# frodik13/gstreamer-vit-tracker

Measured on NVIDIA B200. Metric: 1080p tracked frames/s, higher is better.
Workload: dtype bf16x3 (split bf16 operands, fp32 accumulate)

## Files before the change

gstreamer_vit_tracker_b200/csrc/attention_tc.cu:

```cuda
#include "tc_common.cuh"
#include "vt_internal.h"

namespace vt {

using namespace tc;

constexpr int kDh = 64;
constexpr int kQTile = 128;
constexpr int kKeyChunk = 64;
constexpr int kNChunks = kNTok / kKeyChunk;
constexpr int kQBytes = kQTile * kDh * 2;
constexpr int kKBytes = kNTok * kDh * 2;
constexpr int kVBytes = kDh * kNTok * 2;
constexpr int kPBytes = kQTile * kKeyChunk * 2;
constexpr uint32_t kTmemCols = 512;
constexpr uint32_t kColO = 320;
constexpr uint32_t kColA = 128;
constexpr int kSoftmaxWarps = 16, kSoftmaxThreads = kSoftmaxWarps * 32;
constexpr int kAttThreads = kSoftmaxThreads + 32;
constexpr int kColGroups = kSoftmaxThreads / kQTile;
constexpr int kKeysPerThread = kKeyChunk / kColGroups;

template <int NSPLIT>
struct AttSmem {
    static constexpr int kParts = NSPLIT == 3 ? 2 : 1;
    static constexpr int kQK = kParts * (kQBytes + kKBytes);
    static constexpr int kP = kParts * kPBytes;
    static constexpr int kRegion1 = kQK > kP ? kQK : kP;
    static constexpr int kV = kParts * kVBytes;
    static constexpr int kW2 = kParts * kAttChainW * 128;
    static constexpr int kTotal = kRegion1 + kV + kW2 + 1024;
};

__device__ __forceinline__ void softmax_bar_sync() { asm volatile("bar.sync 1, %0;" ::"n"(kSoftmaxThreads) : "memory"); }

template <int NSPLIT>
__global__ void __launch_bounds__(kAttThreads, 1)
attention_tc_kernel(const __grid_constant__ TcAttentionPlan mp, __nv_bfloat16* __restrict__ out_hi, __nv_bfloat16* __restrict__ out_lo, int D,
                    int heads, int* err, unsigned long long* trace, int dup) {
    const CUtensorMap &mQhi = mp.mQhi, &mQlo = mp.mQlo, &mKhi = mp.mKhi, &mKlo = mp.mKlo, &mVhi = mp.mVhi, &mVlo = mp.mVlo;
    extern __shared__ uint8_t smem_raw[];
    __shared__ __align__(8) uint64_t bar_qk, bar_k1, bar_v, bar_s, p_full[kNChunks], bar_o, bar_w2, bar_a2, bar_o2;
    __shared__ uint32_t tmem_base_s;
    __shared__ float red[kColGroups][kQTile];
    __shared__ unsigned long long* trace_slot;
    using SM = AttSmem<NSPLIT>;
    constexpr int P = SM::kParts;
    uint8_t* smem = reinterpret_cast<uint8_t*>((reinterpret_cast<uintptr_t>(smem_raw) + 1023) & ~uintptr_t(1023));
    uint8_t* sQ = smem;
    uint8_t* sK = smem + P * kQBytes;
    uint8_t* sV = smem + SM::kRegion1;
    uint8_t* sW2 = sV + SM::kV;

    const int tid = threadIdx.x, warp = tid >> 5, lane = tid & 31;
    const bool ctrl = warp == kSoftmaxWarps;
    const int row = (warp & 3) * 32 + lane;
    const int g = (warp >> 2) & 3;
    constexpr int kQTiles = (kNTok + kQTile - 1) / kQTile;
    const int replica = blockIdx.x / kQTiles;
    const bool st_hi = !dup || replica == 0, st_lo = P == 2 && (!dup || replica == 1);
    const bool chain = mp.chain != 0;
    const int q0 = (blockIdx.x % kQTiles) * kQTile, h = blockIdx.y, b = blockIdx.z;
    const int bh = b * heads + h;
    const bool q_ok = q0 + row < kNTok;
    bool ok = true;
    TraceRec tr;
    tr.begin(&trace_slot, trace, 10);

    if (tid == 0) {
        mbar_init(&bar_qk, 1), mbar_init(&bar_k1, 1), mbar_init(&bar_v, 1), mbar_init(&bar_s, 1), mbar_init(&bar_o, 1);
        mbar_init(&bar_w2, 1), mbar_init(&bar_a2, kSoftmaxWarps), mbar_init(&bar_o2, 1);
        for (int c = 0; c < kNChunks; ++c) mbar_init(&p_full[c], kSoftmaxWarps);
        fence_barrier_init();
    }
    if (ctrl) {
        if (elect_one_sync()) {
            tma_prefetch_desc(&mQhi), tma_prefetch_desc(&mKhi), tma_prefetch_desc(&mVhi);
            if (P == 2) tma_prefetch_desc(&mQlo), tma_prefetch_desc(&mKlo), tma_prefetch_desc(&mVlo);
        }
        tmem_alloc(&tmem_base_s, kTmemCols);
        tmem_relinquish();
    }
    tcgen05_fence_before();
    __syncthreads();
    if (chain && ctrl && elect_one_sync()) {
// ... 8 lines not shown
    pdl_wait();
    if (tid == 0) tr.mark(2);
    pdl_launch_dependents();

    if (ctrl) {
        if (elect_one_sync()) {
            constexpr int kHalfK = kNTok / 2, kHalfKBytes = kHalfK * kDh * 2;
            mbar_arrive_expect_tx(&bar_qk, P * (kQBytes + kHalfKBytes));
            tma_load_3d(sQ, &mQhi, &bar_qk, 0, q0, bh);
            tma_load_3d(sK, &mKhi, &bar_qk, 0, 0, bh);
            if (P == 2) tma_load_3d(sQ + kQBytes, &mQlo, &bar_qk, 0, q0, bh), tma_load_3d(sK + kKBytes, &mKlo, &bar_qk, 0, 0, bh);
            mbar_arrive_expect_tx(&bar_k1, P * kHalfKBytes);
            tma_load_3d(sK + kHalfKBytes, &mKhi, &bar_k1, 0, kHalfK, bh);
            if (P == 2) tma_load_3d(sK + kKBytes + kHalfKBytes, &mKlo, &bar_k1, 0, kHalfK, bh);
            mbar_arrive_expect_tx(&bar_v, P * kVBytes);
            for (int c = 0; c < kNChunks; ++c) {
                tma_load_3d(sV + c * (P * kDh * 128), &mVhi, &bar_v, c * kKeyChunk, 0, bh);
                if (P == 2) tma_load_3d(sV + c * (P * kDh * 128) + kDh * 128, &mVlo, &bar_v, c * kKeyChunk, 0, bh);
            }
            ok &= mbar_wait(&bar_qk, 0);
            tcgen05_fence_after();
            const uint64_t dQ = umma_desc_sw128(smem_u32(sQ)), dK = umma_desc_sw128(smem_u32(sK));
            constexpr int kHalf = kNTok / 2;
            constexpr uint32_t idescS = umma_idesc_h<NSPLIT == 2>(kQTile, kHalf);
            constexpr uint64_t kLoQ = kQBytes >> 4, kLoK = kKBytes >> 4, kK2 = (kHalf * 128) >> 4;
#pragma unroll
            for (int half = 0; half < 2; ++half) {
                if (half) {
                    ok &= mbar_wait(&bar_k1, 0);
                    tcgen05_fence_after();
                }
#pragma unroll
                for (int k = 0; k < kDh / 16; ++k) {
                    const uint64_t qh = dQ + 2 * k, kh = dK + 2 * k + half * kK2;
                    umma_bf16(tmem + half * kHalf, qh, kh, idescS, k != 0);
                    if (NSPLIT == 3) {
                        umma_bf16(tmem + half * kHalf, qh, kh + kLoK, idescS, 1);
                        umma_bf16(tmem + half * kHalf, qh + kLoQ, kh, idescS, 1);
                    }
                }
            }
            umma_commit(&bar_s);
            const uint64_t dV = umma_desc_sw128(smem_u32(sV));
            constexpr uint32_t idesc = umma_idesc_h<NSPLIT == 2>(kQTile, kDh), idesc2n = umma_idesc_h<NSPLIT == 2>(kQTile, 2 * kDh);
            constexpr uint64_t kBlkV = (uint64_t)(P * kDh * 128) >> 4;
            ok &= mbar_wait(&bar_v, 0);
            for (int c = 0; c < kNChunks; ++c) {
                ok &= mbar_wait(&p_full[c], 0);
                tcgen05_fence_after();
#pragma unroll
                for (int k = 0; k < kKeyChunk / 16; ++k) {
                    const uint32_t ph = tmem + c * kKeyChunk + k * kKeysPerThread;
                    const uint64_t vh = dV + c * kBlkV + 2 * k;
                    if (NSPLIT == 3) {
                        umma_bf16_ta(tmem + kColO, ph, vh, idesc2n, (c | k) != 0);
                        umma_bf16_ta(tmem + kColO, ph + 8, vh, idesc, 1);
                    } else {
                        umma_bf16_ta(tmem + kColO, ph, vh, idesc, (c | k) != 0);
                    }
                }
            }
            umma_commit(&bar_o);
            if (chain) {
                ok &= mbar_wait(&bar_w2, 0);
                ok &= mbar_wait(&bar_a2, 0);
                tcgen05_fence_after();
                const uint64_t dW = umma_desc_sw128(smem_u32(sW2));
                constexpr uint32_t idescW = umma_idesc_h<NSPLIT == 2>(kQTile, kAttChainW), idescW2 = umma_idesc_h<NSPLIT == 2>(kQTile, 2 * kAttChainW);
#pragma unroll
                for (int k = 0; k < kDh / 16; ++k) {
                    const uint32_t ah = tmem + kColA + k * 16;
                    if (NSPLIT == 3) {
                        umma_bf16_ta(tmem, ah, dW + 2 * k, idescW2, k != 0);
                        umma_bf16_ta(tmem, ah + 8, dW + 2 * k, idescW, 1);
                    } else {
                        umma_bf16_ta(tmem, ah, dW + 2 * k, idescW, k != 0);
                    }
                }
                umma_commit(&bar_o2);
            }
        }
        __syncwarp();
    } else {
        ok &= mbar_wait(&bar_s, 0);
        tcgen05_fence_after();
        if (tid == 0) tr.mark(4);
        const uint32_t lane_addr = tmem + ((uint32_t)((warp & 3) * 32) << 16);
        const float k2 = 1.4426950408889634f / sqrtf((float)kDh);
        float mx = -INFINITY;
        const uint32_t col0 = lane_addr + g * kKeysPerThread;
        uint32_t r[2][16];
        if (q_ok) {
            tmem_ld_32x16_issue(col0, r[0]);
#pragma unroll
            for (int c = 0; c < kNChunks; ++c) {
                tmem_ld_wait(r[c & 1]);
                if (c + 1 < kNChunks) tmem_ld_32x16_issue(col0 + (c + 1) * kKeyChunk, r[(c + 1) & 1]);
#pragma unroll
                for (int j = 0; j < 16; ++j) mx = fmaxf(mx, __uint_as_float(r[c & 1][j]));
            }
            tmem_ld_32x16_issue(col0, r[0]);
        }
        red[g][row] = mx;
        softmax_bar_sync();
        mx = fmaxf(fmaxf(red[0][row], red[1][row]), fmaxf(red[2][row], red[3][row]));
        if (tid == 0) tr.mark(5);
        const float mk = mx * k2;
        float sum = 0.f;
#pragma unroll
        for (int c = 0; c < kNChunks; ++c) {
            uint32_t hi[8], lo[8];
            if (q_ok) {
                tmem_ld_wait(r[c & 1]);
                if (c + 1 < kNChunks) tmem_ld_32x16_issue(col0 + (c + 1) * kKeyChunk, r[(c + 1) & 1]);
#pragma unroll
                for (int j = 0; j < 16; j += 2) {
                    const float e0 = ex2_approx(fmaf(__uint_as_float(r[c & 1][j]), k2, -mk));
                    const float e1 = ex2_approx(fmaf(__uint_as_float(r[c & 1][j + 1]), k2, -mk));
                    sum += e0;
                    sum += e1;
                    split2_h<NSPLIT == 2>(e0, e1, hi[j >> 1], lo[j >> 1]);
                }
            }
            if (q_ok) {
                tmem_st_32x8(col0 + c * kKeyChunk, hi);
                if (P == 2) tmem_st_32x8(col0 + c * kKeyChunk + 8, lo);
                tmem_st_wait();
            }
            tcgen05_fence_before();
            __syncwarp();
            if (lane == 0) mbar_arrive(&p_full[c]);
            if (tid == 0 && c == 0) tr.mark(6);
        }
        if (tid == 0) tr.mark(7);
        red[g][row] = sum;
        softmax_bar_sync();
        sum = (red[0][row] + red[1][row]) + (red[2][row] + red[3][row]);

        ok &= mbar_wait(&bar_o, 0);
        tcgen05_fence_after();
        {
            const float inv = q_ok ? 1.f / sum : 0.f;
            float v[16];
            tmem_ld_32x16(lane_addr + kColO + g * 16, v);
            if (NSPLIT == 3) {
                float hl[16];
                tmem_ld_32x16(lane_addr + kColO + kDh + g * 16, hl);
#pragma unroll
                for (int j = 0; j < 16; ++j) v[j] += hl[j];
            }
            uint32_t hi[8], lo[8];
#pragma unroll
            for (int j = 0; j < 16; j += 2) split2_h<NSPLIT == 2>(v[j] * inv, v[j + 1] * inv, hi[j >> 1], lo[j >> 1]);
            if (chain) {
                tmem_st_32x8(lane_addr + kColA + g * 16, hi);
                if (P == 2) tmem_st_32x8(lane_addr + kColA + g * 16 + 8, lo);
                tmem_st_wait();
            } else {
#pragma unroll
                for (int j = 0; j < 2; ++j) {
                    const int off = row * 128 + (((2 * g + j) ^ (row & 7)) << 4);
                    *reinterpret_cast<uint4*>(smem + off) = make_uint4(hi[4 * j], hi[4 * j + 1], hi[4 * j + 2], hi[4 * j + 3]);
                    if (P == 2) *reinterpret_cast<uint4*>(smem + kPBytes + off) = make_uint4(lo[4 * j], lo[4 * j + 1], lo[4 * j + 2], lo[4 * j + 3]);
                }
            }
        }
        if (chain) {
            tcgen05_fence_before();
            __syncwarp();
            if (lane == 0) mbar_arrive(&bar_a2);
            ok &= mbar_wait(&bar_o2, 0);
            tcgen05_fence_after();
            constexpr int CW = kAttChainW / kColGroups;
            float v[CW];
            tmem_ld_cols(lane_addr + g * CW, v);
            if (NSPLIT == 3) {
                float hl[CW];
                tmem_ld_cols(lane_addr + kAttChainW + g * CW, hl);
#pragma unroll
                for (int j = 0; j < CW; ++j) v[j] += hl[j];
            }
            uint8_t* prow = smem + 2 * kPBytes + ((g * CW) >> 5) * (kQTile * 128) + row * 128;
            const int ch0 = ((g * CW) & 31) >> 2;
#pragma unroll
            for (int q = 0; q < CW / 4; ++q)
                *reinterpret_cast<float4*>(prow + (((ch0 + q) ^ (row & 7)) << 4)) = make_float4(v[4 * q], v[4 * q + 1], v[4 * q + 2], v[4 * q + 3]);
            softmax_bar_sync();
            constexpr int CH = kAttChainW / 4, RPP = kSoftmaxThreads / CH;
#pragma unroll
            for (int i = 0; i < kQTile / RPP; ++i) {
                const int r = tid / CH + RPP * i, c16 = tid % CH, bx = c16 >> 3, ch = c16 & 7;
                if (q0 + r < kNTok) {
                    const float4 val = *reinterpret_cast<const float4*>(smem + 2 * kPBytes + bx * (kQTile * 128) + r * 128 + ((ch ^ (r & 7)) << 4));
                    float* dst = mp.p2 + (int64_t)h * mp.p2_plane + ((int64_t)b * kNTok + q0 + r) * D + replica * kAttChainW + c16 * 4;
                    *reinterpret_cast<float4*>(dst) = val;
                }
            }
        } else {
        softmax_bar_sync();
#pragma unroll
        for (int i = 0; i < 2; ++i) {
            const int r = (tid >> 3) + 64 * i, ch = tid & 7;
            if (q0 + r < kNTok) {
                const int off = r * 128 + ((ch ^ (r & 7)) << 4);
                const int64_t dst = (((int64_t)b * kNTok + q0 + r) * D + h * kDh) * 2 + ch * 16;
                if (st_hi) *reinterpret_cast<uint4*>(reinterpret_cast<uint8_t*>(out_hi) + dst) = *reinterpret_cast<const uint4*>(smem + off);
                if (st_lo) *reinterpret_cast<uint4*>(reinterpret_cast<uint8_t*>(out_lo) + dst) = *reinterpret_cast<const uint4*>(smem + kPBytes + off);
            }
        }
        }
    }
    if (!ok && err) atomicExch(err, 2);
    tcgen05_fence_before();
    __syncthreads();
    if (tid == 0) tr.mark(3);
    if (ctrl) tmem_dealloc(tmem, kTmemCols);
}

bool tc_make_map(CUtensorMap* out, const void* base, int rank, const uint64_t* dims, const uint64_t* strides_bytes, const uint32_t* box);

bool tc_attention_plan_init(TcAttentionPlan* p, const __nv_bfloat16* Qhi, const __nv_bfloat16* Qlo, const __nv_bfloat16* Khi, const __nv_bfloat16* Klo,
                            const __nv_bfloat16* Vthi, const __nv_bfloat16* Vtlo, int batch_heads, __nv_bfloat16* out_hi, __nv_bfloat16* out_lo, int D,
                            int batch) {
    bool ok = true;
    p->out_hi = out_hi, p->out_lo = out_lo, p->D = D;
    p->p2 = nullptr, p->p2_plane = 0, p->chain = 0;
    (void)batch;
    {
        const uint64_t dims[3] = {kDh, kNTok, (uint64_t)batch_heads}, strides[2] = {kDh * 2, (uint64_t)kDh * 2 * kNTok};
        const uint32_t boxq[3] = {kDh, kQTile, 1}, boxk[3] = {kDh, kNTok / 2, 1};
        ok &= tc_make_map(&p->mQhi, Qhi, 3, dims, strides, boxq) && tc_make_map(&p->mQlo, Qlo, 3, dims, strides, boxq);
        ok &= tc_make_map(&p->mKhi, Khi, 3, dims, strides, boxk) && tc_make_map(&p->mKlo, Klo, 3, dims, strides, boxk);
    }
    {
        const uint64_t dims[3] = {kNTok, kDh, (uint64_t)batch_heads}, strides[2] = {kNTok * 2, (uint64_t)kNTok * 2 * kDh};
        const uint32_t box[3] = {kKeyChunk, kDh, 1};
        ok &= tc_make_map(&p->mVhi, Vthi, 3, dims, strides, box) && tc_make_map(&p->mVlo, Vtlo, 3, dims, strides, box);
    }
    return ok;
}

cudaError_t tc_attention_setup() {
    cudaError_t e = cudaFuncSetAttribute(attention_tc_kernel<1>, cudaFuncAttributeMaxDynamicSharedMemorySize, AttSmem<1>::kTotal);
    if (e != cudaSuccess) return e;
    e = cudaFuncSetAttribute(attention_tc_kernel<2>, cudaFuncAttributeMaxDynamicSharedMemorySize, AttSmem<2>::kTotal);
    if (e != cudaSuccess) return e;
    return cudaFuncSetAttribute(attention_tc_kernel<3>, cudaFuncAttributeMaxDynamicSharedMemorySize, AttSmem<3>::kTotal);
}

cudaError_t tc_attention_launch(const TcAttentionPlan& p, int B, int heads, int nsplit, int* err, cudaStream_t s, bool pdl, unsigned long long* trace,
                                int form) {
    if (B <= 0) return cudaSuccess;
    dim3 grid((kNTok + kQTile - 1) / kQTile, heads, B);
    const int ctas = (int)(grid.x * grid.y * grid.z);
    int dup = 0;
    TcAttentionPlan q = p;
    q.chain = 0;
    if (form == VT_ATT_CHAIN) {
        if (!p.p2 || ctas * (p.D / kAttChainW) > kSpreadCtas) return cudaErrorInvalidValue;
        q.chain = 1, grid.x *= p.D / kAttChainW;
    } else if (form == VT_ATT_DUP && nsplit == 3 && ctas * 2 <= kSpreadCtas) {
        dup = 1, grid.x *= 2;
    }
    if (nsplit == 3) return launch_ex(attention_tc_kernel<3>, grid, dim3(kAttThreads), AttSmem<3>::kTotal, s, pdl, 1, q, p.out_hi, p.out_lo, p.D, heads, err, trace, dup);
    if (nsplit == 2) return launch_ex(attention_tc_kernel<2>, grid, dim3(kAttThreads), AttSmem<2>::kTotal, s, pdl, 1, q, p.out_hi, p.out_lo, p.D, heads, err, trace, dup);
    return launch_ex(attention_tc_kernel<1>, grid, dim3(kAttThreads), AttSmem<1>::kTotal, s, pdl, 1, q, p.out_hi, p.out_lo, p.D, heads, err, trace, dup);
}

bool tc_attention_plan_chain(TcAttentionPlan* p, const __nv_bfloat16* Whi, const __nv_bfloat16* Wlo, float* P2, int64_t plane_elems) {
    const uint64_t dims[2] = {(uint64_t)p->D, (uint64_t)p->D}, strides[1] = {(uint64_t)p->D * 2};
    const uint32_t box[2] = {64, kAttChainW};
    const bool ok = tc_make_map(&p->mW2hi, Whi, 2, dims, strides, box) && tc_make_map(&p->mW2lo, Wlo ? Wlo : Whi, 2, dims, strides, box);
    p->p2 = P2, p->p2_plane = plane_elems;
    return ok;
}

}
```

gstreamer_vit_tracker_b200/csrc/tc_common.cuh:

```cuda
#pragma once

#include <cuda.h>
#include <cuda_bf16.h>
#include <cuda_fp16.h>
#include <cuda_runtime.h>
#include <stdint.h>

namespace vt {
namespace tc {

__device__ __forceinline__ uint32_t smem_u32(const void* p) { return (uint32_t)__cvta_generic_to_shared(p); }

__device__ __forceinline__ void mbar_init(uint64_t* bar, uint32_t count) {
    asm volatile("mbarrier.init.shared::cta.b64 [%0], %1;" ::"r"(smem_u32(bar)), "r"(count));
}
__device__ __forceinline__ void fence_barrier_init() { asm volatile("fence.mbarrier_init.release.cluster;" ::: "memory"); }
__device__ __forceinline__ void mbar_arrive_expect_tx(uint64_t* bar, uint32_t bytes) {
    asm volatile("mbarrier.arrive.expect_tx.shared::cta.b64 _, [%0], %1;" ::"r"(smem_u32(bar)), "r"(bytes) : "memory");
}
__device__ __forceinline__ void mbar_arrive(uint64_t* bar) {
    asm volatile("mbarrier.arrive.shared::cta.b64 _, [%0];" ::"r"(smem_u32(bar)) : "memory");
}
__device__ __forceinline__ bool mbar_try_wait(uint64_t* bar, uint32_t parity) {
    uint32_t ok;
// ... 281 lines not shown
    asm volatile(
        "tcgen05.ld.sync.aligned.32x32b.x16.b32 {%0, %1, %2, %3, %4, %5, %6, %7, %8, %9, %10, %11, %12, %13, %14, %15}, [%16];"
        : "=r"(r[0]), "=r"(r[1]), "=r"(r[2]), "=r"(r[3]), "=r"(r[4]), "=r"(r[5]), "=r"(r[6]), "=r"(r[7]), "=r"(r[8]), "=r"(r[9]), "=r"(r[10]),
          "=r"(r[11]), "=r"(r[12]), "=r"(r[13]), "=r"(r[14]), "=r"(r[15])
        : "r"(taddr));
}
__device__ __forceinline__ void tmem_ld_wait(uint32_t (&r)[16]) {
    asm volatile("tcgen05.wait::ld.sync.aligned;"
                 : "+r"(r[0]), "+r"(r[1]), "+r"(r[2]), "+r"(r[3]), "+r"(r[4]), "+r"(r[5]), "+r"(r[6]), "+r"(r[7]), "+r"(r[8]), "+r"(r[9]), "+r"(r[10]),
                   "+r"(r[11]), "+r"(r[12]), "+r"(r[13]), "+r"(r[14]), "+r"(r[15])::"memory");
}
__device__ __forceinline__ void tmem_ld_32x8(uint32_t taddr, float (&v)[8]) {
    uint32_t r[8];
    asm volatile("tcgen05.ld.sync.aligned.32x32b.x8.b32 {%0, %1, %2, %3, %4, %5, %6, %7}, [%8];"
                 : "=r"(r[0]), "=r"(r[1]), "=r"(r[2]), "=r"(r[3]), "=r"(r[4]), "=r"(r[5]), "=r"(r[6]), "=r"(r[7])
                 : "r"(taddr));
    asm volatile("tcgen05.wait::ld.sync.aligned;"
                 : "+r"(r[0]), "+r"(r[1]), "+r"(r[2]), "+r"(r[3]), "+r"(r[4]), "+r"(r[5]), "+r"(r[6]), "+r"(r[7])::"memory");
#pragma unroll
    for (int i = 0; i < 8; ++i) v[i] = __uint_as_float(r[i]);
}
__device__ __forceinline__ void tmem_ld_cols(uint32_t taddr, float (&v)[16]) { tmem_ld_32x16(taddr, v); }
__device__ __forceinline__ void tmem_ld_cols(uint32_t taddr, float (&v)[8]) { tmem_ld_32x8(taddr, v); }
__device__ __forceinline__ float ex2_approx(float x) {
    float y;
    asm("ex2.approx.ftz.f32 %0, %1;" : "=f"(y) : "f"(x));
    return y;
}

__device__ __forceinline__ uint64_t f2_pack(float a, float b) {
    uint64_t r;
    asm("mov.b64 %0, {%1, %2};" : "=l"(r) : "f"(a), "f"(b));
    return r;
}
__device__ __forceinline__ void f2_unpack(uint64_t v, float& a, float& b) { asm("mov.b64 {%0, %1}, %2;" : "=f"(a), "=f"(b) : "l"(v)); }
__device__ __forceinline__ uint64_t f2_fma(uint64_t a, uint64_t b, uint64_t c) {
    uint64_t d;
    asm("fma.rn.f32x2 %0, %1, %2, %3;" : "=l"(d) : "l"(a), "l"(b), "l"(c));
    return d;
}
__device__ __forceinline__ uint64_t f2_mul(uint64_t a, uint64_t b) {
    uint64_t d;
    asm("mul.rn.f32x2 %0, %1, %2;" : "=l"(d) : "l"(a), "l"(b));
    return d;
}
__device__ __forceinline__ uint64_t f2_add(uint64_t a, uint64_t b) {
// ... 35 lines not shown
```

gstreamer_vit_tracker_b200/csrc/tracker_create.cu:

```cuda
#include "tracker_state.h"

namespace vt {

static thread_local char g_err[512] = "";
void set_error(const char* fmt, ...) {
    va_list ap;
    va_start(ap, fmt);
    vsnprintf(g_err, sizeof(g_err), fmt, ap);
    va_end(ap);
}

static std::mutex g_weight_mutex;
static std::map<std::string, std::weak_ptr<WeightSet>> g_weight_cache;

bool frame_is_pinned(const void* p) { return is_pinned(p); }
bool is_pinned(const void* p) {
    cudaPointerAttributes a;
    if (cudaPointerGetAttributes(&a, p) != cudaSuccess) {
        cudaGetLastError();
        return false;
    }
    return a.type == cudaMemoryTypeHost;
}

// ... 324 lines not shown
    VT_TRY(cudaMemset(t->patches_x, 0, sizeof(float) * B * kNTx * kPatchK));
    VT_TRY(cudaMemset(t->patches_z, 0, sizeof(float) * kNTz * kPatchK));
    if (t->debug_capture) VT_TRY(cudaMalloc(&t->d_dbg, sizeof(float) * (size_t)(t->depth + 1) * B * kNTok * D));
    t->nsplit = cfg->gemm_mode == VT_GEMM_TCGEN05_BF16X3 ? 3 : (cfg->gemm_mode == VT_GEMM_TCGEN05_BF16 ? 1 : (cfg->gemm_mode == VT_GEMM_TCGEN05_FP16 ? 2 : 0));
    t->f16 = t->nsplit == 2;
    if (t->nsplit) {
        if (D % 64 || Hd % 64 || C % 64) {
            set_error("the tcgen05 path needs D, hidden and head_ch to be multiples of 64 (D=%zu hidden=%zu head_ch=%zu)", D, Hd, C);
            return fail(VT_ERR_WEIGHTS);
        }
        VT_TRY(tc_gemm_setup());
        VT_TRY(tc_gemm_as_setup());
        VT_TRY(cudaDeviceGetAttribute(&t->sm_count, cudaDevAttrMultiProcessorCount, cfg->device));
        if (const char* e = getenv("VT_B200_AS_ROWS")) t->as_rows = atoi(e);
        if (const char* e = getenv("VT_B200_TP_ROWS")) t->tp_rows = atoi(e);
        t->as_mlp = !getenv("VT_B200_NO_AS_MLP");
        t->fuse_ln = D / 64 <= 8 && !getenv("VT_B200_NO_FUSE_LN");
        t->pdl = !getenv("VT_B200_NO_PDL");
        t->spread_ok = !getenv("VT_B200_NO_SPREAD");
        if (const char* e = getenv("VT_B200_UNCHAIN_N")) t->unchain_n = atoi(e);
        t->chain_mlp = t->fuse_ln && D <= 192 && !getenv("VT_B200_NO_CHAIN");
        if (t->chain_mlp) VT_TRY(cudaMalloc(&t->Pbuf, sizeof(float) * (Hd / 64) * B * kNTok * D));
        t->att_chain_ok = t->chain_mlp && t->fuse_ln && D / t->heads == 64 && (int)(Hd / 64) >= t->heads && t->nsplit && !getenv("VT_B200_NO_ATT_CHAIN");
        t->split_k = t->chain_mlp && Hd / 64 >= 4 && (C == 64 || C == 128) && !getenv("VT_B200_NO_SPLITK");
        if (t->split_k) {
            VT_TRY(cudaMalloc(&t->Phead, sizeof(float) * 9 * B * kNTx * C));
            VT_TRY(cudaMalloc(&t->d_cand, sizeof(float) * B * 16 * 8));
            VT_TRY(cudaMalloc(&t->d_counters, sizeof(unsigned) * B));
            VT_TRY(cudaMemset(t->d_counters, 0, sizeof(unsigned) * B));
        }
        {
            std::lock_guard<std::mutex> lock(t->wset->split_mutex);
            if (!t->wset->w_hi) {
                const size_t nw = t->n_weights;
                VT_TRY(cudaMalloc(&t->wset->w_hi, nw * 2));
                VT_TRY(cudaMalloc(&t->wset->w_lo, nw * 2));
                VT_TRY(launch_split_bf16(t->d_weights, t->wset->w_hi, t->wset->w_lo, nw, t->stream));
                VT_TRY(cudaStreamSynchronize(t->stream));
            }
            t->w_hi = t->wset->w_hi, t->w_lo = t->wset->w_lo;
            if (t->f16) {
                if (!t->wset->w_f16) {
                    VT_TRY(cudaMalloc(&t->wset->w_f16, t->n_weights * 2));
                    VT_TRY(launch_split_bf16(t->d_weights, t->wset->w_f16, nullptr, t->n_weights, t->stream));
                    VT_TRY(cudaStreamSynchronize(t->stream));
                }
// ... 151 lines not shown
```

gstreamer_vit_tracker_b200/csrc/tracker_frame.cu:

```cuda
#include "tracker_state.h"

extern "C" int vt_glyph_rows(int ch, uint8_t rows[7]);

namespace vt {

__global__ void gather_template_kernel(float* __restrict__ X, const float* __restrict__ Zemb, const int32_t* __restrict__ slots, int D,
                                       uint32_t* __restrict__ ln_hi, uint32_t* __restrict__ ln_lo, const uint32_t* __restrict__ zln_hi,
                                       const uint32_t* __restrict__ zln_lo, unsigned long long* stamp) {
    tc::pdl_launch_dependents();
    const int bi = blockIdx.y;
    const int n = kNTz * D;
    const size_t so = (size_t)slots[bi] * n, xo = (size_t)bi * kNTok * D;
    for (int i = blockIdx.x * blockDim.x + threadIdx.x; i < n; i += gridDim.x * blockDim.x) {
        X[xo + i] = Zemb[so + i];
        if (ln_hi && i < n / 2) {
            ln_hi[xo / 2 + i] = zln_hi[so / 2 + i];
            if (ln_lo) ln_lo[xo / 2 + i] = zln_lo[so / 2 + i];
        }
    }
    tc::pdl_wait();
    if (stamp && threadIdx.x == 0 && blockIdx.x == 0 && blockIdx.y == 0) *stamp = device_time_ns();
}

static GemmArgs gemm_args(const float* A, int64_t lda, const float* W, const float* bias, float* C, int64_t ldc, int M, int N, int K) {
// ... 72 lines not shown
            pp.args.kb_per_split = kPatchK / 64 / 2, patch_np = 2;
            VT_LAUNCH(tc_gemm_launch(pp, n * kNTx, ns, s, pdl));
        } else {
            VT_LAUNCH(tc_gemm_launch(t->plan_patch_x, n * kNTx, ns, s, pdl));
        }
        if (t->split_k) {
            ReduceLnArgs r{};
            r.P = t->Pbuf, r.np = patch_np, r.p_stride = (int64_t)t->maxT * kNTx * D, r.bias = t->patch_b, r.add = t->pos_x, r.add_period = kNTx;
            r.X = t->X, r.M = n * kNTx, r.D = D, r.period = kNTx, r.x_rows = kNTok, r.x_row_off = kNTz;
            r.ln_g = t->blk[0].ln1_g, r.ln_b = t->blk[0].ln1_b, r.ln_hi = t->ln_hi, r.ln_lo = LO(t->ln_lo), r.ln_rows = kNTok, r.ln_row_off = kNTz;
            VT_LAUNCH(launch_reduce_ln(r, s, pdl));
        }
        if (t->debug_capture) VT_CUDA(cudaMemcpyAsync(t->d_dbg, t->X, sizeof(float) * M * D, cudaMemcpyDeviceToDevice, s));
        for (int l = 0; l < t->depth; ++l) {
            const BlockW& b = t->blk[l];
            const vt_tracker::BlockPlans& p = t->plans[l];
            if (!fuse) VT_LAUNCH(launch_layernorm_split(t->X, D, b.ln1_g, b.ln1_b, t->ln_hi, LO(t->ln_lo), M, D, 1 << 30, 0, 0, s, pdl));
            const bool as_form = t->as_rows > 0 && M >= t->as_rows;
            const bool tp_mcast = t->tp_rows > 0 && M >= t->tp_rows;
            if (as_form && tc_gemm_as_supported(p.qkv))
                VT_LAUNCH(tc_gemm_as_launch(p.qkv, M, ns, s, pdl, t->sm_count));
            else
                VT_LAUNCH(tc_gemm_launch(p.qkv, M, ns, s, pdl, spread));
            const bool att_chain = spread && t->att_chain_ok && n * t->heads * 3 * (D / kAttChainW) <= kSpreadCtas;
            if (t->tc_attention)
                VT_LAUNCH(tc_attention_launch(att_chain ? p.att : t->plan_att, n, t->heads, ns, t->d_tc_err, s, pdl, t->d_trace,
                                              att_chain ? VT_ATT_CHAIN : (spread ? VT_ATT_DUP : VT_ATT_PLAIN)));
            else
                VT_LAUNCH(launch_attention(t->QKV, nullptr, t->att_hi, LO(t->att_lo), n, D, t->heads, s));
            if (att_chain) {
                ReduceLnArgs r{};
                r.P = t->Pbuf, r.np = t->heads, r.p_stride = (int64_t)t->maxT * kNTok * D, r.bias = b.proj_b, r.add = t->X, r.add_period = 0;
                r.X = t->X, r.M = M, r.D = D, r.period = kNTok, r.x_rows = kNTok, r.x_row_off = 0;
                r.ln_g = b.ln2_g, r.ln_b = b.ln2_b, r.ln_hi = t->ln_hi, r.ln_lo = LO(t->ln_lo), r.ln_rows = kNTok, r.ln_row_off = 0;
                VT_LAUNCH(launch_reduce_ln(r, s, pdl));
            } else {
                VT_LAUNCH(tc_gemm_launch(p.proj, M, ns, s, pdl && t->tc_attention, spread && !tp_mcast, tp_mcast));
            }
            if (!fuse) VT_LAUNCH(launch_layernorm_split(t->X, D, b.ln2_g, b.ln2_b, t->ln_hi, LO(t->ln_lo), M, D, 1 << 30, 0, 0, s, pdl));
            const bool as_mlp = as_form && t->chain_mlp && t->as_mlp && tc_gemm_as_mlp_supported(p.fc1, ns);
            const bool chain = as_mlp || (t->chain_mlp && n < t->unchain_n);
            int planes = (int)(Hd / 64);
            if (as_mlp) {
                VT_LAUNCH(tc_gemm_as_mlp_launch(p.fc1, M, s, pdl, t->sm_count, &planes, t->fuse_ln ? &p.fc2 : nullptr));
            } else if (chain) {
                VT_LAUNCH(tc_gemm_launch(p.fc1, M, ns, s, pdl, spread));
            } else {
                TcGemmPlan fc1 = p.fc1;
                fc1.args.chain_n = 0, fc1.args.o_mode = 1;
                if (as_form && tc_gemm_as_supported(fc1))
// ... 801 lines not shown
```

gstreamer_vit_tracker_b200/csrc/tracker_state.h:

```cpp
#pragma once

#include <math.h>
#include <stdarg.h>
#include <stdio.h>
#include <stdlib.h>
#include <string.h>

#include <sys/stat.h>

#include <algorithm>
#include <atomic>
#include <chrono>
#include <map>
#include <memory>
#include <mutex>
#include <string>
#include <vector>

#include "tc_common.cuh"
#include "vt_internal.h"

namespace vt {

struct BlockW {
// ... 93 lines not shown
    bool chain_mlp = false;
    float* Pbuf = nullptr;
    bool split_k = false;
    float *Phead = nullptr, *d_cand = nullptr;
    unsigned* d_counters = nullptr;
    bool pdl = true;
    bool spread_ok = true;
    int unchain_n = kUnchainTargets;
    int sm_count = 148;
    int as_rows = 1024;
    bool as_mlp = true;
    int tp_rows = 0;
    bool counted = false;
    bool tc_attention = false;
    TcAttentionPlan plan_att;
    int* d_tc_err = nullptr;
    unsigned long long* d_trace = nullptr;
    TcGemmPlan plan_patch_x, plan_patch_z, plan_head;
    struct BlockPlans {
        TcGemmPlan qkv, proj, fc1, fc2;
        TcAttentionPlan att;
    };
    bool att_chain_ok = false;
    std::vector<BlockPlans> plans;

    std::map<int, cudaGraphExec_t> graphs;
    int kernels_per_frame = 0;
    uint64_t kernel_launches = 0, frames = 0, h2d_bytes = 0, d2h_bytes = 0;

    static constexpr int kQueue = 2;
    struct Slot {
        uint8_t* frame = nullptr;
        size_t len = 0;
        bool mirrored = false, pageable = false;
        size_t hud_bytes = 0;
        std::chrono::steady_clock::time_point t_submit;
    } q[kQueue];
    int q_head = 0, q_count = 0;
    DeviceResult* h_blk[kQueue] = {nullptr, nullptr};
    cudaEvent_t q_done[kQueue] = {nullptr, nullptr};
    bool in_flight = false;
    uint8_t* inflight_frame = nullptr;
    std::chrono::steady_clock::time_point t_submit;

    bool hostprof = false;
    double hp[8] = {0, 0, 0, 0, 0, 0, 0, 0};
// ... 32 lines not shown
```

gstreamer_vit_tracker_b200/csrc/vt_internal.h:

```cpp
#pragma once

#include <cuda.h>
#include <cuda_bf16.h>
#include <cuda_fp16.h>
#include <cuda_runtime.h>
#include <stdint.h>

#include <string>
#include <vector>

#include "vt_tracker.h"

namespace vt {

constexpr int kNTz = 64;
constexpr int kNTx = 256;
constexpr int kNTok = 320;
constexpr int kPatchK = 768;
constexpr int kSearch = 256;
constexpr int kTemplate = 128;
constexpr int kMap = 16;
constexpr int kWindow = 120;
constexpr int kMaxCmds = 32;

// ... 244 lines not shown
};
struct TcGemmPlan {
    TcMaps maps;
    TcGemmArgs args;
    bool mcast_ok;
    int bn;
};
bool tc_plan_init(TcGemmPlan* p, const __nv_bfloat16* Ahi, const __nv_bfloat16* Alo, uint64_t a_rows, const __nv_bfloat16* Whi,
                  const __nv_bfloat16* Wlo, int N, int K, int conv_feat, int conv_batch, int bn = 64);
bool tc_plan_chain(TcGemmPlan* p, const __nv_bfloat16* W2hi, const __nv_bfloat16* W2lo, int N2, float* P, uint64_t rows, uint64_t batch);
TcOut tc_out(void* base, int elem_bytes, int64_t cols, int rows, int heads, int batch, int planes);
TcOut tc_out_vt(void* base, int tokens, int heads, int batch);
bool tc_resid_map(CUtensorMap* out, const float* base, uint64_t rows, uint64_t cols);
cudaError_t tc_gemm_setup();
constexpr int kSpreadCtas = 132;
cudaError_t tc_gemm_launch(const TcGemmPlan& p, int M, int nsplit, cudaStream_t s, bool pdl, bool spread = false, bool mcast_ln = false);
cudaError_t tc_gemm_as_setup();
bool tc_gemm_as_supported(const TcGemmPlan& p);
cudaError_t tc_gemm_as_launch(const TcGemmPlan& p, int M, int nsplit, cudaStream_t s, bool pdl, int sm_count);
bool tc_gemm_as_mlp_supported(const TcGemmPlan& p, int nsplit);
cudaError_t tc_gemm_as_mlp_launch(const TcGemmPlan& p, int M, cudaStream_t s, bool pdl, int sm_count, int* planes, const TcGemmPlan* fc2 = nullptr);
struct TcAttentionPlan {
    CUtensorMap mQhi, mQlo, mKhi, mKlo, mVhi, mVlo;
    CUtensorMap mW2hi, mW2lo;
    __nv_bfloat16 *out_hi, *out_lo;
    float* p2;
    int64_t p2_plane;
    int D, chain;
};
bool tc_attention_plan_init(TcAttentionPlan* p, const __nv_bfloat16* Qhi, const __nv_bfloat16* Qlo, const __nv_bfloat16* Khi, const __nv_bfloat16* Klo,
                            const __nv_bfloat16* Vthi, const __nv_bfloat16* Vtlo, int batch_heads, __nv_bfloat16* out_hi, __nv_bfloat16* out_lo, int D,
                            int batch);
bool tc_attention_plan_chain(TcAttentionPlan* p, const __nv_bfloat16* Whi, const __nv_bfloat16* Wlo, float* P2, int64_t plane_elems);
cudaError_t tc_attention_setup();
enum { VT_ATT_PLAIN = 0, VT_ATT_DUP = 1, VT_ATT_CHAIN = 2 };
constexpr int kAttChainW = 32;
cudaError_t tc_attention_launch(const TcAttentionPlan& p, int B, int heads, int nsplit, int* err, cudaStream_t s, bool pdl,
                                unsigned long long* trace = nullptr, int form = VT_ATT_PLAIN);
cudaError_t launch_split_bf16(const float* x, __nv_bfloat16* hi, __nv_bfloat16* lo, size_t n, cudaStream_t s);

}
```

Baseline: 3191.

## Add 64-row query tile variant of chained attention kernel for more CTAs

```diff
diff --git a/gstreamer_vit_tracker_b200/csrc/attention_tc.cu b/gstreamer_vit_tracker_b200/csrc/attention_tc.cu
--- a/gstreamer_vit_tracker_b200/csrc/attention_tc.cu
+++ b/gstreamer_vit_tracker_b200/csrc/attention_tc.cu
@@ -6,24 +6,24 @@
 using namespace tc;
 
 constexpr int kDh = 64;
-constexpr int kQTile = 128;
 constexpr int kKeyChunk = 64;
 constexpr int kNChunks = kNTok / kKeyChunk;
-constexpr int kQBytes = kQTile * kDh * 2;
 constexpr int kKBytes = kNTok * kDh * 2;
 constexpr int kVBytes = kDh * kNTok * 2;
-constexpr int kPBytes = kQTile * kKeyChunk * 2;
 constexpr uint32_t kTmemCols = 512;
 constexpr uint32_t kColO = 320;
 constexpr uint32_t kColA = 128;
 constexpr int kSoftmaxWarps = 16, kSoftmaxThreads = kSoftmaxWarps * 32;
 constexpr int kAttThreads = kSoftmaxThreads + 32;
-constexpr int kColGroups = kSoftmaxThreads / kQTile;
-constexpr int kKeysPerThread = kKeyChunk / kColGroups;
-
-template <int NSPLIT>
+
+template <int NSPLIT, int QT>
 struct AttSmem {
     static constexpr int kParts = NSPLIT == 3 ? 2 : 1;
+    static constexpr int kQBytes = QT * kDh * 2;
+    static constexpr int kPBytes = QT * kKeyChunk * 2;
+    static constexpr int kQTiles = (kNTok + QT - 1) / QT;
+    static constexpr int kColGroups = kSoftmaxThreads / QT;
+    static constexpr int kKeys = kKeyChunk / kColGroups;
     static constexpr int kQK = kParts * (kQBytes + kKBytes);
     static constexpr int kP = kParts * kPBytes;
     static constexpr int kRegion1 = kQK > kP ? kQK : kP;
@@ -34,18 +34,34 @@
 
 __device__ __forceinline__ void softmax_bar_sync() { asm volatile("bar.sync 1, %0;" ::"n"(kSoftmaxThreads) : "memory"); }
 
-template <int NSPLIT>
+template <int QT, int N>
+__device__ __forceinline__ void ld_row_issue(uint32_t a, uint32_t (&r)[N]) {
+    if constexpr (QT == 64) tmem_ld_16x2_x8_issue(a, r); else tmem_ld_32x16_issue(a, r);
+}
+template <int QT, int N>
+__device__ __forceinline__ void ld_row(uint32_t a, float (&v)[N]) {
+    if constexpr (QT == 64) tmem_ld_16x2(a, v); else tmem_ld_cols(a, v);
+}
+template <int QT, int N>
+__device__ __forceinline__ void st_row(uint32_t a, const uint32_t (&r)[N]) {
+    if constexpr (QT == 64) tmem_st_16x2_x4(a, r); else tmem_st_32x8(a, r);
+}
+
+template <int NSPLIT, int QT>
 __global__ void __launch_bounds__(kAttThreads, 1)
 attention_tc_kernel(const __grid_constant__ TcAttentionPlan mp, __nv_bfloat16* __restrict__ out_hi, __nv_bfloat16* __restrict__ out_lo, int D,
                     int heads, int* err, unsigned long long* trace, int dup) {
-    const CUtensorMap &mQhi = mp.mQhi, &mQlo = mp.mQlo, &mKhi = mp.mKhi, &mKlo = mp.mKlo, &mVhi = mp.mVhi, &mVlo = mp.mVlo;
+    using SM = AttSmem<NSPLIT, QT>;
+    constexpr bool kQ64 = QT == 64;
+    constexpr int P = SM::kParts, kQBytes = SM::kQBytes, kPBytes = SM::kPBytes, kQTiles = SM::kQTiles;
+    constexpr int kColGroups = SM::kColGroups, kKeys = SM::kKeys;
+    const CUtensorMap &mQhi = kQ64 ? mp.mQ64hi : mp.mQhi, &mQlo = kQ64 ? mp.mQ64lo : mp.mQlo;
+    const CUtensorMap &mKhi = mp.mKhi, &mKlo = mp.mKlo, &mVhi = mp.mVhi, &mVlo = mp.mVlo;
     extern __shared__ uint8_t smem_raw[];
     __shared__ __align__(8) uint64_t bar_qk, bar_k1, bar_v, bar_s, p_full[kNChunks], bar_o, bar_w2, bar_a2, bar_o2;
     __shared__ uint32_t tmem_base_s;
-    __shared__ float red[kColGroups][kQTile];
+    __shared__ float red[kColGroups][QT];
     __shared__ unsigned long long* trace_slot;
-    using SM = AttSmem<NSPLIT>;
-    constexpr int P = SM::kParts;
     uint8_t* smem = reinterpret_cast<uint8_t*>((reinterpret_cast<uintptr_t>(smem_raw) + 1023) & ~uintptr_t(1023));
     uint8_t* sQ = smem;
     uint8_t* sK = smem + P * kQBytes;
@@ -54,13 +70,13 @@
 
     const int tid = threadIdx.x, warp = tid >> 5, lane = tid & 31;
     const bool ctrl = warp == kSoftmaxWarps;
-    const int row = (warp & 3) * 32 + lane;
+    const int row = kQ64 ? (warp & 3) * 16 + (lane & 15) : (warp & 3) * 32 + lane;
     const int g = (warp >> 2) & 3;
-    constexpr int kQTiles = (kNTok + kQTile - 1) / kQTile;
+    const int cg = kQ64 ? 2 * g + (lane >> 4) : g;
     const int replica = blockIdx.x / kQTiles;
     const bool st_hi = !dup || replica == 0, st_lo = P == 2 && (!dup || replica == 1);
-    const bool chain = mp.chain != 0;
-    const int q0 = (blockIdx.x % kQTiles) * kQTile, h = blockIdx.y, b = blockIdx.z;
+    const bool chain = kQ64 || mp.chain != 0;
+    const int q0 = (blockIdx.x % kQTiles) * QT, h = blockIdx.y, b = blockIdx.z;
     const int bh = b * heads + h;
     const bool q_ok = q0 + row < kNTok;
     bool ok = true;
@@ -115,7 +131,7 @@
             tcgen05_fence_after();
             const uint64_t dQ = umma_desc_sw128(smem_u32(sQ)), dK = umma_desc_sw128(smem_u32(sK));
             constexpr int kHalf = kNTok / 2;
-            constexpr uint32_t idescS = umma_idesc_h<NSPLIT == 2>(kQTile, kHalf);
+            constexpr uint32_t idescS = umma_idesc_h<NSPLIT == 2>(QT, kHalf);
             constexpr uint64_t kLoQ = kQBytes >> 4, kLoK = kKBytes >> 4, kK2 = (kHalf * 128) >> 4;
 #pragma unroll
             for (int half = 0; half < 2; ++half) {
@@ -135,7 +151,7 @@
             }
             umma_commit(&bar_s);
             const uint64_t dV = umma_desc_sw128(smem_u32(sV));
-            constexpr uint32_t idesc = umma_idesc_h<NSPLIT == 2>(kQTile, kDh), idesc2n = umma_idesc_h<NSPLIT == 2>(kQTile, 2 * kDh);
+            constexpr uint32_t idesc = umma_idesc_h<NSPLIT == 2>(QT, kDh), idesc2n = umma_idesc_h<NSPLIT == 2>(QT, 2 * kDh);
             constexpr uint64_t kBlkV = (uint64_t)(P * kDh * 128) >> 4;
             ok &= mbar_wait(&bar_v, 0);
             for (int c = 0; c < kNChunks; ++c) {
@@ -143,7 +159,7 @@
                 tcgen05_fence_after();
 #pragma unroll
                 for (int k = 0; k < kKeyChunk / 16; ++k) {
-                    const uint32_t ph = tmem + c * kKeyChunk + k * kKeysPerThread;
+                    const uint32_t ph = tmem + c * kKeyChunk + k * 16;
                     const uint64_t vh = dV + c * kBlkV + 2 * k;
                     if (NSPLIT == 3) {
                         umma_bf16_ta(tmem + kColO, ph, vh, idesc2n, (c | k) != 0);
@@ -159,7 +175,7 @@
                 ok &= mbar_wait(&bar_a2, 0);
                 tcgen05_fence_after();
                 const uint64_t dW = umma_desc_sw128(smem_u32(sW2));
-                constexpr uint32_t idescW = umma_idesc_h<NSPLIT == 2>(kQTile, kAttChainW), idescW2 = umma_idesc_h<NSPLIT == 2>(kQTile, 2 * kAttChainW);
+                constexpr uint32_t idescW = umma_idesc_h<NSPLIT == 2>(QT, kAttChainW), idescW2 = umma_idesc_h<NSPLIT == 2>(QT, 2 * kAttChainW);
 #pragma unroll
                 for (int k = 0; k < kDh / 16; ++k) {
                     const uint32_t ah = tmem + kColA + k * 16;
@@ -181,33 +197,34 @@
         const uint32_t lane_addr = tmem + ((uint32_t)((warp & 3) * 32) << 16);
         const float k2 = 1.4426950408889634f / sqrtf((float)kDh);
         float mx = -INFINITY;
-        const uint32_t col0 = lane_addr + g * kKeysPerThread;
-        uint32_t r[2][16];
+        const uint32_t col0 = lane_addr + g * 16;
+        uint32_t r[2][kKeys];
         if (q_ok) {
-            tmem_ld_32x16_issue(col0, r[0]);
+            ld_row_issue<QT>(col0, r[0]);
 #pragma unroll
             for (int c = 0; c < kNChunks; ++c) {
                 tmem_ld_wait(r[c & 1]);
-                if (c + 1 < kNChunks) tmem_ld_32x16_issue(col0 + (c + 1) * kKeyChunk, r[(c + 1) & 1]);
-#pragma unroll
-                for (int j = 0; j < 16; ++j) mx = fmaxf(mx, __uint_as_float(r[c & 1][j]));
-            }
-            tmem_ld_32x16_issue(col0, r[0]);
-        }
-        red[g][row] = mx;
+                if (c + 1 < kNChunks) ld_row_issue<QT>(col0 + (c + 1) * kKeyChunk, r[(c + 1) & 1]);
+#pragma unroll
+                for (int j = 0; j < kKeys; ++j) mx = fmaxf(mx, __uint_as_float(r[c & 1][j]));
+            }
+            ld_row_issue<QT>(col0, r[0]);
+        }
+        red[cg][row] = mx;
         softmax_bar_sync();
         mx = fmaxf(fmaxf(red[0][row], red[1][row]), fmaxf(red[2][row], red[3][row]));
+        if constexpr (kColGroups == 8) mx = fmaxf(mx, fmaxf(fmaxf(red[4][row], red[5][row]), fmaxf(red[6][row], red[7][row])));
         if (tid == 0) tr.mark(5);
         const float mk = mx * k2;
         float sum = 0.f;
 #pragma unroll
         for (int c = 0; c < kNChunks; ++c) {
-            uint32_t hi[8], lo[8];
+            uint32_t hi[kKeys / 2], lo[kKeys / 2];
             if (q_ok) {
                 tmem_ld_wait(r[c & 1]);
-                if (c + 1 < kNChunks) tmem_ld_32x16_issue(col0 + (c + 1) * kKeyChunk, r[(c + 1) & 1]);
-#pragma unroll
-                for (int j = 0; j < 16; j += 2) {
+                if (c + 1 < kNChunks) ld_row_issue<QT>(col0 + (c + 1) * kKeyChunk, r[(c + 1) & 1]);
+#pragma unroll
+                for (int j = 0; j < kKeys; j += 2) {
                     const float e0 = ex2_approx(fmaf(__uint_as_float(r[c & 1][j]), k2, -mk));
                     const float e1 = ex2_approx(fmaf(__uint_as_float(r[c & 1][j + 1]), k2, -mk));
                     sum += e0;
@@ -216,8 +233,8 @@
                 }
             }
             if (q_ok) {
-                tmem_st_32x8(col0 + c * kKeyChunk, hi);
-                if (P == 2) tmem_st_32x8(col0 + c * kKeyChunk + 8, lo);
+                st_row<QT>(col0 + c * kKeyChunk, hi);
+                if (P == 2) st_row<QT>(col0 + c * kKeyChunk + 8, lo);
                 tmem_st_wait();
             }
             tcgen05_fence_before();
@@ -226,30 +243,31 @@
             if (tid == 0 && c == 0) tr.mark(6);
         }
         if (tid == 0) tr.mark(7);
-        red[g][row] = sum;
+        red[cg][row] = sum;
         softmax_bar_sync();
         sum = (red[0][row] + red[1][row]) + (red[2][row] + red[3][row]);
+        if constexpr (kColGroups == 8) sum += (red[4][row] + red[5][row]) + (red[6][row] + red[7][row]);
 
         ok &= mbar_wait(&bar_o, 0);
         tcgen05_fence_after();
         {
             const float inv = q_ok ? 1.f / sum : 0.f;
-            float v[16];
-            tmem_ld_32x16(lane_addr + kColO + g * 16, v);
+            float v[kKeys];
+            ld_row<QT>(lane_addr + kColO + g * 16, v);
             if (NSPLIT == 3) {
-                float hl[16];
-                tmem_ld_32x16(lane_addr + kColO + kDh + g * 16, hl);
-#pragma unroll
-                for (int j = 0; j < 16; ++j) v[j] += hl[j];
-            }
-            uint32_t hi[8], lo[8];
-#pragma unroll
-            for (int j = 0; j < 16; j += 2) split2_h<NSPLIT == 2>(v[j] * inv, v[j + 1] * inv, hi[j >> 1], lo[j >> 1]);
+                float hl[kKeys];
+                ld_row<QT>(lane_addr + kColO + kDh + g * 16, hl);
+#pragma unroll
+                for (int j = 0; j < kKeys; ++j) v[j] += hl[j];
+            }
+            uint32_t hi[kKeys / 2], lo[kKeys / 2];
+#pragma unroll
+            for (int j = 0; j < kKeys; j += 2) split2_h<NSPLIT == 2>(v[j] * inv, v[j + 1] * inv, hi[j >> 1], lo[j >> 1]);
             if (chain) {
-                tmem_st_32x8(lane_addr + kColA + g * 16, hi);
-                if (P == 2) tmem_st_32x8(lane_addr + kColA + g * 16 + 8, lo);
+                st_row<QT>(lane_addr + kColA + g * 16, hi);
+                if (P == 2) st_row<QT>(lane_addr + kColA + g * 16 + 8, lo);
                 tmem_st_wait();
-            } else {
+            } else if constexpr (!kQ64) {
 #pragma unroll
                 for (int j = 0; j < 2; ++j) {
                     const int off = row * 128 + (((2 * g + j) ^ (row & 7)) << 4);
@@ -266,30 +284,30 @@
             tcgen05_fence_after();
             constexpr int CW = kAttChainW / kColGroups;
             float v[CW];
-            tmem_ld_cols(lane_addr + g * CW, v);
+            ld_row<QT>(lane_addr + g * (kAttChainW / 4), v);
             if (NSPLIT == 3) {
                 float hl[CW];
-                tmem_ld_cols(lane_addr + kAttChainW + g * CW, hl);
+                ld_row<QT>(lane_addr + kAttChainW + g * (kAttChainW / 4), hl);
 #pragma unroll
                 for (int j = 0; j < CW; ++j) v[j] += hl[j];
             }
-            uint8_t* prow = smem + 2 * kPBytes + ((g * CW) >> 5) * (kQTile * 128) + row * 128;
-            const int ch0 = ((g * CW) & 31) >> 2;
+            uint8_t* prow = smem + 2 * kPBytes + ((cg * CW) >> 5) * (QT * 128) + row * 128;
+            const int ch0 = ((cg * CW) & 31) >> 2;
 #pragma unroll
             for (int q = 0; q < CW / 4; ++q)
                 *reinterpret_cast<float4*>(prow + (((ch0 + q) ^ (row & 7)) << 4)) = make_float4(v[4 * q], v[4 * q + 1], v[4 * q + 2], v[4 * q + 3]);
             softmax_bar_sync();
             constexpr int CH = kAttChainW / 4, RPP = kSoftmaxThreads / CH;
 #pragma unroll
-            for (int i = 0; i < kQTile / RPP; ++i) {
+            for (int i = 0; i < QT / RPP; ++i) {
                 const int r = tid / CH + RPP * i, c16 = tid % CH, bx = c16 >> 3, ch = c16 & 7;
                 if (q0 + r < kNTok) {
-                    const float4 val = *reinterpret_cast<const float4*>(smem + 2 * kPBytes + bx * (kQTile * 128) + r * 128 + ((ch ^ (r & 7)) << 4));
+                    const float4 val = *reinterpret_cast<const float4*>(smem + 2 * kPBytes + bx * (QT * 128) + r * 128 + ((ch ^ (r & 7)) << 4));
                     float* dst = mp.p2 + (int64_t)h * mp.p2_plane + ((int64_t)b * kNTok + q0 + r) * D + replica * kAttChainW + c16 * 4;
                     *reinterpret_cast<float4*>(dst) = val;
                 }
             }
-        } else {
+        } else if constexpr (!kQ64) {
         softmax_bar_sync();
 #pragma unroll
         for (int i = 0; i < 2; ++i) {
@@ -321,8 +339,9 @@
     (void)batch;
     {
         const uint64_t dims[3] = {kDh, kNTok, (uint64_t)batch_heads}, strides[2] = {kDh * 2, (uint64_t)kDh * 2 * kNTok};
-        const uint32_t boxq[3] = {kDh, kQTile, 1}, boxk[3] = {kDh, kNTok / 2, 1};
+        const uint32_t boxq[3] = {kDh, 128, 1}, boxq64[3] = {kDh, 64, 1}, boxk[3] = {kDh, kNTok / 2, 1};
         ok &= tc_make_map(&p->mQhi, Qhi, 3, dims, strides, boxq) && tc_make_map(&p->mQlo, Qlo, 3, dims, strides, boxq);
+        ok &= tc_make_map(&p->mQ64hi, Qhi, 3, dims, strides, boxq64) && tc_make_map(&p->mQ64lo, Qlo, 3, dims, strides, boxq64);
         ok &= tc_make_map(&p->mKhi, Khi, 3, dims, strides, boxk) && tc_make_map(&p->mKlo, Klo, 3, dims, strides, boxk);
     }
     {
@@ -333,31 +352,44 @@
     return ok;
 }
 
+template <int NSPLIT, int QT>
+static cudaError_t att_set_smem() {
+    return cudaFuncSetAttribute(attention_tc_kernel<NSPLIT, QT>, cudaFuncAttributeMaxDynamicSharedMemorySize, AttSmem<NSPLIT, QT>::kTotal);
+}
 cudaError_t tc_attention_setup() {
-    cudaError_t e = cudaFuncSetAttribute(attention_tc_kernel<1>, cudaFuncAttributeMaxDynamicSharedMemorySize, AttSmem<1>::kTotal);
-    if (e != cudaSuccess) return e;
-    e = cudaFuncSetAttribute(attention_tc_kernel<2>, cudaFuncAttributeMaxDynamicSharedMemorySize, AttSmem<2>::kTotal);
-    if (e != cudaSuccess) return e;
-    return cudaFuncSetAttribute(attention_tc_kernel<3>, cudaFuncAttributeMaxDynamicSharedMemorySize, AttSmem<3>::kTotal);
+    const cudaError_t e[6] = {att_set_smem<1, 128>(), att_set_smem<2, 128>(), att_set_smem<3, 128>(),
+                              att_set_smem<1, 64>(),  att_set_smem<2, 64>(),  att_set_smem<3, 64>()};
+    for (cudaError_t x : e)
+        if (x != cudaSuccess) return x;
+    return cudaSuccess;
+}
+
+template <int QT>
+static cudaError_t att_launch(dim3 grid, const TcAttentionPlan& q, int heads, int nsplit, int* err, cudaStream_t s, bool pdl, unsigned long long* trace,
+                              int dup) {
+    if (nsplit == 3)
+        return launch_ex(attention_tc_kernel<3, QT>, grid, dim3(kAttThreads), AttSmem<3, QT>::kTotal, s, pdl, 1, q, q.out_hi, q.out_lo, q.D, heads, err, trace, dup);
+    if (nsplit == 2)
+        return launch_ex(attention_tc_kernel<2, QT>, grid, dim3(kAttThreads), AttSmem<2, QT>::kTotal, s, pdl, 1, q, q.out_hi, q.out_lo, q.D, heads, err, trace, dup);
+    return launch_ex(attention_tc_kernel<1, QT>, grid, dim3(kAttThreads), AttSmem<1, QT>::kTotal, s, pdl, 1, q, q.out_hi, q.out_lo, q.D, heads, err, trace, dup);
 }
 
 cudaError_t tc_attention_launch(const TcAttentionPlan& p, int B, int heads, int nsplit, int* err, cudaStream_t s, bool pdl, unsigned long long* trace,
                                 int form) {
     if (B <= 0) return cudaSuccess;
-    dim3 grid((kNTok + kQTile - 1) / kQTile, heads, B);
+    const bool q64 = form == VT_ATT_CHAIN_Q64;
+    dim3 grid(q64 ? AttSmem<3, 64>::kQTiles : AttSmem<3, 128>::kQTiles, heads, B);
     const int ctas = (int)(grid.x * grid.y * grid.z);
     int dup = 0;
     TcAttentionPlan q = p;
     q.chain = 0;
-    if (form == VT_ATT_CHAIN) {
+    if (form == VT_ATT_CHAIN || q64) {
         if (!p.p2 || ctas * (p.D / kAttChainW) > kSpreadCtas) return cudaErrorInvalidValue;
         q.chain = 1, grid.x *= p.D / kAttChainW;
     } else if (form == VT_ATT_DUP && nsplit == 3 && ctas * 2 <= kSpreadCtas) {
         dup = 1, grid.x *= 2;
     }
-    if (nsplit == 3) return launch_ex(attention_tc_kernel<3>, grid, dim3(kAttThreads), AttSmem<3>::kTotal, s, pdl, 1, q, p.out_hi, p.out_lo, p.D, heads, err, trace, dup);
-    if (nsplit == 2) return launch_ex(attention_tc_kernel<2>, grid, dim3(kAttThreads), AttSmem<2>::kTotal, s, pdl, 1, q, p.out_hi, p.out_lo, p.D, heads, err, trace, dup);
-    return launch_ex(attention_tc_kernel<1>, grid, dim3(kAttThreads), AttSmem<1>::kTotal, s, pdl, 1, q, p.out_hi, p.out_lo, p.D, heads, err, trace, dup);
+    return q64 ? att_launch<64>(grid, q, heads, nsplit, err, s, pdl, trace, dup) : att_launch<128>(grid, q, heads, nsplit, err, s, pdl, trace, dup);
 }
 
 bool tc_attention_plan_chain(TcAttentionPlan* p, const __nv_bfloat16* Whi, const __nv_bfloat16* Wlo, float* P2, int64_t plane_elems) {
diff --git a/gstreamer_vit_tracker_b200/csrc/tc_common.cuh b/gstreamer_vit_tracker_b200/csrc/tc_common.cuh
--- a/gstreamer_vit_tracker_b200/csrc/tc_common.cuh
+++ b/gstreamer_vit_tracker_b200/csrc/tc_common.cuh
@@ -327,6 +327,33 @@
 }
 __device__ __forceinline__ void tmem_ld_cols(uint32_t taddr, float (&v)[16]) { tmem_ld_32x16(taddr, v); }
 __device__ __forceinline__ void tmem_ld_cols(uint32_t taddr, float (&v)[8]) { tmem_ld_32x8(taddr, v); }
+
+__device__ __forceinline__ void tmem_ld_16x2_x8_issue(uint32_t taddr, uint32_t (&r)[8]) {
+    asm volatile("tcgen05.ld.sync.aligned.16x32bx2.x8.b32 {%0, %1, %2, %3, %4, %5, %6, %7}, [%8], 8;"
+                 : "=r"(r[0]), "=r"(r[1]), "=r"(r[2]), "=r"(r[3]), "=r"(r[4]), "=r"(r[5]), "=r"(r[6]), "=r"(r[7])
+                 : "r"(taddr));
+}
+__device__ __forceinline__ void tmem_ld_wait(uint32_t (&r)[8]) {
+    asm volatile("tcgen05.wait::ld.sync.aligned;" : "+r"(r[0]), "+r"(r[1]), "+r"(r[2]), "+r"(r[3]), "+r"(r[4]), "+r"(r[5]), "+r"(r[6]), "+r"(r[7])::"memory");
+}
+__device__ __forceinline__ void tmem_ld_16x2(uint32_t taddr, float (&v)[8]) {
+    uint32_t r[8];
+    tmem_ld_16x2_x8_issue(taddr, r);
+    tmem_ld_wait(r);
+#pragma unroll
+    for (int i = 0; i < 8; ++i) v[i] = __uint_as_float(r[i]);
+}
+__device__ __forceinline__ void tmem_ld_16x2(uint32_t taddr, float (&v)[4]) {
+    uint32_t r[4];
+    asm volatile("tcgen05.ld.sync.aligned.16x32bx2.x4.b32 {%0, %1, %2, %3}, [%4], 4;" : "=r"(r[0]), "=r"(r[1]), "=r"(r[2]), "=r"(r[3]) : "r"(taddr));
+    asm volatile("tcgen05.wait::ld.sync.aligned;" : "+r"(r[0]), "+r"(r[1]), "+r"(r[2]), "+r"(r[3])::"memory");
+#pragma unroll
+    for (int i = 0; i < 4; ++i) v[i] = __uint_as_float(r[i]);
+}
+__device__ __forceinline__ void tmem_st_16x2_x4(uint32_t taddr, const uint32_t (&r)[4]) {
+    asm volatile("tcgen05.st.sync.aligned.16x32bx2.x4.b32 [%0], 4, {%1, %2, %3, %4};" ::"r"(taddr), "r"(r[0]), "r"(r[1]), "r"(r[2]), "r"(r[3])
+                 : "memory");
+}
 __device__ __forceinline__ float ex2_approx(float x) {
     float y;
     asm("ex2.approx.ftz.f32 %0, %1;" : "=f"(y) : "f"(x));
diff --git a/gstreamer_vit_tracker_b200/csrc/tracker_create.cu b/gstreamer_vit_tracker_b200/csrc/tracker_create.cu
--- a/gstreamer_vit_tracker_b200/csrc/tracker_create.cu
+++ b/gstreamer_vit_tracker_b200/csrc/tracker_create.cu
@@ -370,6 +370,7 @@
         t->chain_mlp = t->fuse_ln && D <= 192 && !getenv("VT_B200_NO_CHAIN");
         if (t->chain_mlp) VT_TRY(cudaMalloc(&t->Pbuf, sizeof(float) * (Hd / 64) * B * kNTok * D));
         t->att_chain_ok = t->chain_mlp && t->fuse_ln && D / t->heads == 64 && (int)(Hd / 64) >= t->heads && t->nsplit && !getenv("VT_B200_NO_ATT_CHAIN");
+        t->att_q64 = !getenv("VT_B200_ATT_Q128");
         t->split_k = t->chain_mlp && Hd / 64 >= 4 && (C == 64 || C == 128) && !getenv("VT_B200_NO_SPLITK");
         if (t->split_k) {
             VT_TRY(cudaMalloc(&t->Phead, sizeof(float) * 9 * B * kNTx * C));
diff --git a/gstreamer_vit_tracker_b200/csrc/tracker_frame.cu b/gstreamer_vit_tracker_b200/csrc/tracker_frame.cu
--- a/gstreamer_vit_tracker_b200/csrc/tracker_frame.cu
+++ b/gstreamer_vit_tracker_b200/csrc/tracker_frame.cu
@@ -118,10 +118,11 @@
                 VT_LAUNCH(tc_gemm_as_launch(p.qkv, M, ns, s, pdl, t->sm_count));
             else
                 VT_LAUNCH(tc_gemm_launch(p.qkv, M, ns, s, pdl, spread));
-            const bool att_chain = spread && t->att_chain_ok && n * t->heads * 3 * (D / kAttChainW) <= kSpreadCtas;
+            const bool att_q64 = spread && t->att_chain_ok && t->att_q64 && n * t->heads * 5 * (D / kAttChainW) <= kSpreadCtas;
+            const bool att_chain = att_q64 || (spread && t->att_chain_ok && n * t->heads * 3 * (D / kAttChainW) <= kSpreadCtas);
             if (t->tc_attention)
                 VT_LAUNCH(tc_attention_launch(att_chain ? p.att : t->plan_att, n, t->heads, ns, t->d_tc_err, s, pdl, t->d_trace,
-                                              att_chain ? VT_ATT_CHAIN : (spread ? VT_ATT_DUP : VT_ATT_PLAIN)));
+                                              att_q64 ? VT_ATT_CHAIN_Q64 : att_chain ? VT_ATT_CHAIN : (spread ? VT_ATT_DUP : VT_ATT_PLAIN)));
             else
                 VT_LAUNCH(launch_attention(t->QKV, nullptr, t->att_hi, LO(t->att_lo), n, D, t->heads, s));
             if (att_chain) {
diff --git a/gstreamer_vit_tracker_b200/csrc/tracker_state.h b/gstreamer_vit_tracker_b200/csrc/tracker_state.h
--- a/gstreamer_vit_tracker_b200/csrc/tracker_state.h
+++ b/gstreamer_vit_tracker_b200/csrc/tracker_state.h
@@ -139,6 +139,7 @@
         TcAttentionPlan att;
     };
     bool att_chain_ok = false;
+    bool att_q64 = true;
     std::vector<BlockPlans> plans;
 
     std::map<int, cudaGraphExec_t> graphs;
diff --git a/gstreamer_vit_tracker_b200/csrc/vt_internal.h b/gstreamer_vit_tracker_b200/csrc/vt_internal.h
--- a/gstreamer_vit_tracker_b200/csrc/vt_internal.h
+++ b/gstreamer_vit_tracker_b200/csrc/vt_internal.h
@@ -290,6 +290,7 @@
 cudaError_t tc_gemm_as_mlp_launch(const TcGemmPlan& p, int M, cudaStream_t s, bool pdl, int sm_count, int* planes, const TcGemmPlan* fc2 = nullptr);
 struct TcAttentionPlan {
     CUtensorMap mQhi, mQlo, mKhi, mKlo, mVhi, mVlo;
+    CUtensorMap mQ64hi, mQ64lo;
     CUtensorMap mW2hi, mW2lo;
     __nv_bfloat16 *out_hi, *out_lo;
     float* p2;
@@ -301,7 +302,7 @@
                             int batch);
 bool tc_attention_plan_chain(TcAttentionPlan* p, const __nv_bfloat16* Whi, const __nv_bfloat16* Wlo, float* P2, int64_t plane_elems);
 cudaError_t tc_attention_setup();
-enum { VT_ATT_PLAIN = 0, VT_ATT_DUP = 1, VT_ATT_CHAIN = 2 };
+enum { VT_ATT_PLAIN = 0, VT_ATT_DUP = 1, VT_ATT_CHAIN = 2, VT_ATT_CHAIN_Q64 = 3 };
 constexpr int kAttChainW = 32;
 cudaError_t tc_attention_launch(const TcAttentionPlan& p, int B, int heads, int nsplit, int* err, cudaStream_t s, bool pdl,
                                 unsigned long long* trace = nullptr, int form = VT_ATT_PLAIN);
```

Result: faster. 3308, median of 6 (+3.7%).
